# Sabarna07-tech/Multimodal-RAG-for-Image-Text-Search

Measured on AMD Instinct MI355X. Metric: CLIP img-embeds/sec/GPU; kNN queries/sec on 1M×512 at top-k=10, 1/2/4/8 GPUs, higher is better.
Workload: dtype fp16 MFMA scan + f64 exact rescore; 1 GPU; BASELINE config 3 (N=1) / config 4 (N>1): brute-force cosine top-10, 1M x 512 rows per GPU, 1000-query batch; rows_per_gpu=1048576, total_rows=1048576, dim=512, top_k=10, parallelism=row-sharded x1, uncertified_queries_last_step=0, searches_in_flight=2

## Files before the change

multimodal-rag-for-image-text-search_amd/csrc/knn.hip:

```cpp
#include <algorithm>
#include <cstdlib>
#include <mutex>
#include <shared_mutex>
#include <type_traits>
#include <utility>
#include <vector>

#include "common.h"
#include "knn_generic.h"

#define AS1 __attribute__((address_space(1)))
#define AS3 __attribute__((address_space(3)))

namespace {

constexpr int TILE_ROWS = 64;
constexpr int SCAN_WAVES = 8;
constexpr int SCAN_THREADS = SCAN_WAVES * 64;
constexpr int QPW = 32;
constexpr int QPG = SCAN_WAVES * QPW;
constexpr int MAX_MERGE_ENTRIES = 4096;
constexpr int MAX_K = 256;
constexpr int MERGE_THREADS = 256;
#ifndef MRAG_SAMPLE_STRIDE
#define MRAG_SAMPLE_STRIDE 16
#endif
constexpr int SAMPLE_STRIDE = MRAG_SAMPLE_STRIDE;

constexpr double EPS_F16 = 1.05e-3;

struct ScanParams {
  const _Float16* x16;
  const int32_t* labels;
  const _Float16* q16;
  int ntiles, qgroups, splits, Qp, label_filter;
  float* part_s;
  int32_t* part_i;
  const int32_t* fail_list;
  const int32_t* fail_cnt;
  const float* thresh;
  int32_t* cand_cnt;
  int32_t* cand;
  int ccap;
  uint32_t* theta;
  int sample_tiles, sample_stride;
  int k;
  float* part_tau;
};

template <int KL>
__device__ __forceinline__ void list_insert(float (&ls)[KL], int (&li)[KL], float s, int r) {
  float cs = s;
  int cr = r;
#pragma unroll
  for (int j = 0; j < KL; ++j) {
    const bool sw = cs > ls[j];
    const float ts = ls[j];
    const int tr = li[j];
    ls[j] = sw ? cs : ts;
    li[j] = sw ? cr : tr;
    cs = sw ? ts : cs;
    cr = sw ? tr : cr;
  }
}

template <int KL>
__device__ __forceinline__ void list_insert_par(float (&ls)[KL], int (&li)[KL], float s, int r) {
  bool c[KL];
#pragma unroll
  for (int j = 0; j < KL; ++j) c[j] = s > ls[j];
  float ns[KL];
  int ni[KL];
  ns[0] = c[0] ? s : ls[0];
  ni[0] = c[0] ? r : li[0];
#pragma unroll
  for (int j = 1; j < KL; ++j) {
    ns[j] = c[j] ? (c[j - 1] ? ls[j - 1] : s) : ls[j];
    ni[j] = c[j] ? (c[j - 1] ? li[j - 1] : r) : li[j];
  }
#pragma unroll
  for (int j = 0; j < KL; ++j) {
    ls[j] = ns[j];
    li[j] = ni[j];
  }
}

__device__ __forceinline__ void glds_x4(const void* gsrc, uint32_t lds_addr) {
  unsigned keep;
  asm volatile(
      "s_mov_b32 %0, m0\n\ts_mov_b32 m0, %2\n\ts_nop 0\n\tglobal_load_lds_dwordx4 %1, off\n\ts_mov_b32 m0, %0"
      : "=&s"(keep)
      : "v"(gsrc), "s"(lds_addr)
      : "memory");
}
__device__ __forceinline__ void glds_x4_saddr(uint32_t voff, const void* sbase, uint32_t lds_addr) {
  unsigned keep;
  asm volatile(
      "s_mov_b32 %0, m0\n\ts_mov_b32 m0, %3\n\ts_nop 0\n\tglobal_load_lds_dwordx4 %1, %2\n\ts_mov_b32 m0, %0"
      : "=&s"(keep)
      : "v"(voff), "s"(sbase), "s"(lds_addr)
// ... 281 lines not shown
    } else {
      qg = b % p.qgroups;
      split = b / p.qgroups;
    }
  }
  const int slot0 = qg * QPG3 + w * QPW3 + c16;

  half8 qf[KSTEPS][QB];
#pragma unroll
  for (int kk = 0; kk < KSTEPS; ++kk)
#pragma unroll
    for (int qb = 0; qb < QB; ++qb)
      qf[kk][qb] = *(const half8*)(p.q16 + (size_t)(slot0 + 16 * qb) * DP + kk * 32 + g4 * 8);
#pragma unroll
  for (int kk = 0; kk < KSTEPS; ++kk)
#pragma unroll
    for (int qb = 0; qb < QB; ++qb) asm volatile("" ::"a"(qf[kk][qb]));

  float ls[QB][KL3];
  int li[QB][KL3];
  float theta_f[QB], published[QB];
  float thr[QB];
  uint32_t theta_next[QB];
#pragma unroll
  for (int qb = 0; qb < QB; ++qb) {
#pragma unroll
    for (int j = 0; j < KL3; ++j) {
      ls[qb][j] = -INFINITY;
      li[qb][j] = -1;
    }
    theta_f[qb] = -INFINITY;
    thr[qb] = -INFINITY;
    published[qb] = -INFINITY;
    theta_next[qb] = 0u;
  }
  uint32_t* const theta_q = p.theta + slot0;
  const bool may_publish = p.k <= KL3;
  const int lab_lo = p.label_filter == MRAG_LABEL_ANY ? 0 : p.label_filter;
  const uint32_t lab_span = p.label_filter == MRAG_LABEL_ANY ? 0x7fffffffu : 0u;

  const int offA0_init = c16 * ROW_BYTES + 16 * (g4 ^ c16);

  f32x4 acc[2][4][QB];
#pragma unroll
  for (int i = 0; i < 4; ++i)
#pragma unroll
    for (int j = 0; j < QB; ++j) {
      acc[1][i][j] = f32x4{-INFINITY, -INFINITY, -INFINITY, -INFINITY};
      acc[0][i][j] = f32x4{};
    }

  int my_tiles = (split < p.ntiles) ? (p.ntiles - 1 - split) / p.splits + 1 : 0;
  int tstep = p.splits;
  if constexpr (MODE == 1) {
    my_tiles = min(my_tiles, p.sample_tiles);
    tstep = p.splits * p.sample_stride;
  }
  float smax[QB];
#pragma unroll
  for (int qb = 0; qb < QB; ++qb) smax[qb] = -INFINITY;

  auto stage_piece = [&](int buf, int tile, int i, int lane_t) {
    const char* gt = (const char*)p.x16 + (size_t)tile * TILE_BYTES;
    const unsigned piece = w * GLDS_PER_WAVE + i;
    const unsigned P = piece * 64 + (unsigned)lane_t;
    const unsigned row = P / CPR;
    const unsigned pos = P - row * CPR;
    const unsigned c = pos ^ (row & 15);
    glds_x4(gt + row * ROW_BYTES + c * 16, lds_base + buf * TILE_BYTES + piece * 1024);
  };
  auto stage_labels = [&](int buf, int tile) {
    if (w == 0) glds_x1(p.labels + (size_t)tile * TILE_ROWS + lane, lds_base + LBL_OFF + buf * TILE_ROWS * 4);
  };

  int prow = 0;
#ifdef MRAG_K7_STAMPS
  unsigned long long st_sum[7] = {0, 0, 0, 0, 0, 0, 0}, st_mid = 0;
#endif
  auto epi_group = [&](auto g_c, auto y_c) {
    constexpr int G = decltype(g_c)::value;
    constexpr int Y = decltype(y_c)::value;
    constexpr int qb = G >> 2, rb = G & 3;
    f32x4& av = acc[Y][rb][qb];
    float gm;
    asm("v_max3_f32 %0, %1, %2, %3\n\tv_max_f32 %0, %0, %4"
        : "=&v"(gm)
        : "v"(av[0]), "v"(av[1]), "v"(av[2]), "v"(av[3]));
    if constexpr (MODE == 1) {
      float sm = smax[qb];
      asm volatile("v_max_f32 %0, %0, %1" : "+v"(sm) : "v"(gm));
      smax[qb] = sm;
    } else {
      if (__builtin_expect(__any(gm > thr[qb]), 0)) {
#ifdef MRAG_K7_STAMPS
        const unsigned long long fire_t0 = __builtin_amdgcn_s_memtime();
#endif
#pragma unroll
        for (int r = 0; r < 4; ++r) {
          const float sv = av[r];
          if (sv > fmaxf(ls[qb][KL3 - 1], theta_f[qb]))
            list_insert_par<KL3>(ls[qb], li[qb], sv, prow + 16 * rb + r);
        }
        if (may_publish && li[qb][KL3 - 1] >= 0 && ls[qb][KL3 - 1] > published[qb]) {
          published[qb] = ls[qb][KL3 - 1];
          __hip_atomic_fetch_max(theta_q + 16 * qb, mrag_f2ord(published[qb]), __ATOMIC_RELAXED,
                                 __HIP_MEMORY_SCOPE_AGENT);
        }
        thr[qb] = fmaxf(ls[qb][KL3 - 1], theta_f[qb]);
#ifdef MRAG_K7_STAMPS
        st_sum[5] += 1;
        st_sum[6] += __builtin_amdgcn_s_memtime() - fire_t0;
#endif
      }
    }
  };

  constexpr int NA = QB == 4 ? 5 : 4;
  half8 a[NA];
  const int offA0 = offA0_init;
  auto read_a = [&](const char* tb, int kk, int rb) {
    a[(4 * kk + rb) % NA] =
        *(const half8*)(tb + ((offA0 ^ ((kk & 3) << 6)) + (kk >> 2) * 256 + rb * 16 * ROW_BYTES));
  };

  uint32_t m0_keep = 0;
#ifdef MRAG_K7_STAMPS
  unsigned long long st_end[3] = {0, 0, 0};
#endif
  auto end_of_tile = [&](bool wait_part) {
    if (!wait_part) {
#ifdef MRAG_K7_STAMPS
      st_end[0] = __builtin_amdgcn_s_memtime();
#endif
      if constexpr (CPR == 64 && QB == 4) asm volatile("s_mov_b32 m0, %0" ::"s"(m0_keep));
    }
    if (wait_part) {
      asm volatile("s_waitcnt vmcnt(0)" ::: "memory");
      if constexpr (MODE == 0) {
        if (may_publish) {
#pragma unroll
          for (int qb = 0; qb < QB; ++qb) {
            if (theta_next[qb] != 0) theta_f[qb] = fmaxf(theta_f[qb], mrag_ord2f(theta_next[qb]));
            thr[qb] = fmaxf(ls[qb][KL3 - 1], theta_f[qb]);
            asm volatile("" : "+v"(theta_f[qb]), "+v"(thr[qb]));
          }
        }
      }
#ifdef MRAG_K7_STAMPS
      st_end[1] = __builtin_amdgcn_s_memtime();
#endif
      __syncthreads();
#ifdef MRAG_K7_STAMPS
      st_end[2] = __builtin_amdgcn_s_memtime();
#endif
    }
  };

  auto tile_body = [&](auto x_c, int it) {
    constexpr int X = decltype(x_c)::value;
    constexpr int Y = 1 - X;
    K7_STAMP(st0);
    const int tile = split + it * tstep;
    const bool has_next = it + 1 < my_tiles;
    const int ntile = has_next ? tile + tstep : tile;
    const char* gw = (const char*)p.x16 + (size_t)ntile * TILE_BYTES + (size_t)w * GLDS_PER_WAVE * ROW_BYTES;
    uint32_t ldsw = lds_base + Y * TILE_BYTES + w * GLDS_PER_WAVE * 1024;
    asm volatile("" : "+s"(gw), "+s"(ldsw));
    if constexpr (MODE == 0) {
      if (may_publish) {
#pragma unroll
        for (int qb = 0; qb < QB; ++qb)
          theta_next[qb] = __hip_atomic_load(theta_q + 16 * qb, __ATOMIC_RELAXED, __HIP_MEMORY_SCOPE_AGENT);
      }
    }
    const char* tb = smem + X * TILE_BYTES;
    int lane_t = lane;
    uint32_t lane16 = lane * 16;
    asm volatile("" : "+v"(lane_t), "+v"(lane16));
    uint32_t voff = 0;
    if constexpr (CPR == 64 && QB == 4) asm volatile("s_mov_b32 %0, m0" : "=s"(m0_keep));
#pragma unroll
    for (int n = 0; n < NA; ++n) read_a(tb, n >> 2, n & 3);
    stage_labels(Y, ntile);
    constexpr int KLAB = KSTEPS / 2 - 1;
    int lab_v = 0;
    uint64_t tile_mask = ~0ull;
    if constexpr (QB == 1) {
#pragma unroll
      for (int i = 0; i < GLDS_PER_WAVE; ++i) stage_piece(Y, ntile, i, lane_t);
      static_for<KSTEPS>([&](auto kk_c) {
        constexpr int kk = decltype(kk_c)::value;
        static_for<4>([&](auto rb_c) {
          constexpr int rb = decltype(rb_c)::value;
          if constexpr (kk == 0)
            mfma16_ab0(acc[X][rb][0], a[(4 * kk + rb) % NA], qf[kk][0]);
          else
            mfma16_ab(acc[X][rb][0], a[(4 * kk + rb) % NA], qf[kk][0]);
          if constexpr (kk + 1 < KSTEPS) read_a(tb, kk + 1, rb);
          if constexpr (kk == 0) epi_group(std::integral_constant<int, rb>{}, std::integral_constant<int, Y>{});
          __builtin_amdgcn_sched_barrier(0);
        });
      });
    } else static_for<KSTEPS>([&](auto kk_c) {
      constexpr int kk = decltype(kk_c)::value;
      constexpr int g0 = (kk * NGROUPS + KSTEPS - 1) / KSTEPS;
      constexpr int g1 = ((kk + 1) * NGROUPS + KSTEPS - 1) / KSTEPS;
      static_for<16>([&](auto j_c) {
        constexpr int j = decltype(j_c)::value;
        constexpr int rb = j >> 2, qb = j & 3;
        constexpr int n = 4 * kk + rb;
        if constexpr (kk == 0)
          mfma16_ab0(acc[X][rb][qb], a[n % NA], qf[kk][qb]);
        else
          mfma16_ab(acc[X][rb][qb], a[n % NA], qf[kk][qb]);
        if constexpr ((j & 3) == 3) {
          if constexpr (n + NA < 4 * KSTEPS) read_a(tb, (n + NA) >> 2, (n + NA) & 3);
        } else if constexpr ((j & 3) == 1) {
          constexpr int pc = FRONT * kk + (j >> 2);
          if constexpr (CPR == 64 && (j >> 2) < FRONT && pc < GLDS_PER_WAVE) {
            voff = (lane16 ^ (uint32_t)(pc << 4)) + (uint32_t)(pc * 1024);
            asm volatile("s_mov_b32 m0, %1" : "+v"(voff) : "s"(ldsw + pc * 1024));
          }
          static_assert(KLAB * FRONT >= GLDS_PER_WAVE, "label slots must follow the DMA k-steps");
          if constexpr (kk == KLAB && j == 1) lab_v = ((const int*)(smem + LBL_OFF + X * TILE_ROWS * 4))[lane];
          if constexpr (kk == KLAB + 1 && j == 1) tile_mask = __ballot((uint32_t)(lab_v - lab_lo) <= lab_span);
        } else if constexpr ((j & 3) == 2) {
          constexpr int pc = FRONT * kk + (j >> 2);
          if constexpr ((j >> 2) < FRONT && pc < GLDS_PER_WAVE) {
            if constexpr (CPR == 64)
              asm volatile("global_load_lds_dwordx4 %0, %1" ::"v"(voff), "s"(gw) : "memory");
            else
              stage_piece(Y, ntile, pc, lane_t);
          }
        } else if constexpr ((j & 3) == 0) {
          if constexpr (g0 + (j >> 2) < g1)
            epi_group(std::integral_constant<int, g0 + (j >> 2)>{}, std::integral_constant<int, Y>{});
        }
#ifdef MRAG_K7_STAMPS
        if constexpr (kk == (GLDS_PER_WAVE + FRONT - 1) / FRONT - 1 && j == 15) st_mid = __builtin_amdgcn_s_memtime();
#endif
        __builtin_amdgcn_sched_barrier(0);
      });
    });
    end_of_tile(false);
    if constexpr (QB == 1) {
      lab_v = ((const int*)(smem + LBL_OFF + X * TILE_ROWS * 4))[lane];
      tile_mask = __ballot((uint32_t)(lab_v - lab_lo) <= lab_span);
    }
    if (tile_mask != ~0ull) {
      mfma16_guard(acc[X]);
      const uint64_t lm = tile_mask >> (4 * g4);
#pragma unroll
      for (int rb = 0; rb < 4; ++rb)
#pragma unroll
        for (int r = 0; r < 4; ++r) {
          const bool ok = (lm >> (16 * rb + r)) & 1ull;
#pragma unroll
          for (int qb = 0; qb < QB; ++qb) acc[X][rb][qb][r] = ok ? acc[X][rb][qb][r] : -INFINITY;
        }
    }
    prow = tile * TILE_ROWS + 4 * g4;
    end_of_tile(true);
#ifdef MRAG_K7_STAMPS
    if constexpr (QB == 4) {
      st_sum[0] += st_mid - st0;
      st_sum[1] += st_end[0] - st_mid;
    } else {
      st_sum[1] += st_end[0] - st0;
    }
    st_sum[2] += st_end[1] - st_end[0];
    st_sum[3] += st_end[2] - st_end[1];
    st_sum[4] += 1;
#endif
  };

  if constexpr (MODE == 0) {
    if (!may_publish) {
#pragma unroll
      for (int qb = 0; qb < QB; ++qb) {
        const uint32_t t0 = __hip_atomic_load(theta_q + 16 * qb, __ATOMIC_RELAXED, __HIP_MEMORY_SCOPE_AGENT);
        if (t0 != 0) theta_f[qb] = mrag_ord2f(t0);
        thr[qb] = theta_f[qb];
      }
    }
  }
  if (my_tiles > 0) {
#pragma unroll
    for (int i = 0; i < GLDS_PER_WAVE; ++i) stage_piece(0, split, i, lane);
    stage_labels(0, split);
    asm volatile("s_waitcnt vmcnt(0)" ::: "memory");
    __syncthreads();
    for (int it = 0; it < my_tiles; it += 2) {
      tile_body(std::integral_constant<int, 0>{}, it);
      if (it + 1 < my_tiles) tile_body(std::integral_constant<int, 1>{}, it + 1);
    }
    if (my_tiles & 1) {
      static_for<NGROUPS>([&](auto g_c) { epi_group(g_c, std::integral_constant<int, 0>{}); });
    } else {
      static_for<NGROUPS>([&](auto g_c) { epi_group(g_c, std::integral_constant<int, 1>{}); });
    }
  }
#ifdef MRAG_K7_STAMPS
  if constexpr (MODE == 0) {
    const int wid = blockIdx.x * SCAN2_WAVES + w;
    if (lane == 0 && wid < K7_MAXWAVES)
      for (int i = 0; i < 7; ++i) g_k7_stamps[(size_t)wid * K7_NSTAMP + i] = st_sum[i];
  }
#endif

  if constexpr (MODE == 1) {
#pragma unroll
    for (int qb = 0; qb < QB; ++qb) {
      p.part_s[((size_t)split * p.Qp + slot0 + 16 * qb) * 4 + g4] = smax[qb];
    }
    return;
  }
#pragma unroll
  for (int qb = 0; qb < QB; ++qb) {
    float fs[8];
    int fi[8];
#pragma unroll
    for (int j = 0; j < 8; ++j) {
      fs[j] = j < KL3 ? ls[qb][j] : -INFINITY;
      fi[j] = j < KL3 ? li[qb][j] : -1;
    }
    float tau = li[qb][KL3 - 1] >= 0 ? ls[qb][KL3 - 1] : -INFINITY;
#pragma unroll
    for (int o = 16; o < 64; o += 16) {
#pragma unroll
      for (int j = 0; j < KL3; ++j) {
        const float ps = __shfl_xor(ls[qb][j], o);
        const int pi = __shfl_xor(li[qb][j], o);
        if (pi >= 0 && ps > fs[7]) list_insert<8>(fs, fi, ps, pi);
      }
      const int plast = __shfl_xor(li[qb][KL3 - 1], o);
      const float pl = __shfl_xor(ls[qb][KL3 - 1], o);
      if (plast >= 0) tau = fmaxf(tau, pl);
    }
    if (g4 == 0) {
      const int slot = slot0 + 16 * qb;
      float* os = p.part_s + ((size_t)split * p.Qp + slot) * 8;
      int32_t* oi = p.part_i + ((size_t)split * p.Qp + slot) * 8;
#pragma unroll
      for (int j = 0; j < 8; ++j) {
        os[j] = fs[j];
        oi[j] = fi[j];
      }
      if (fi[7] >= 0) tau = fmaxf(tau, fs[7]);
      p.part_tau[(size_t)split * p.Qp + slot] = tau;
    }
  }
}

constexpr float THETA_SEED_MARGIN = (float)(2.5 * EPS_F16);
__global__ __launch_bounds__(64) void theta_init_kernel(const float* __restrict__ smax, int nvals, int Qp, int k,
                                                        uint32_t* __restrict__ theta) {
  constexpr int PER_LANE = 16;
  const int q = blockIdx.x, lane = threadIdx.x;
  float v[PER_LANE];
  const int splits = nvals / 4;
#pragma unroll
  for (int t = 0; t < 4; ++t) {
    const int sp = lane + 64 * t;
    const f32x4 x = sp < splits ? *(const f32x4*)(smax + ((size_t)sp * Qp + q) * 4)
                                : f32x4{-INFINITY, -INFINITY, -INFINITY, -INFINITY};
#pragma unroll
    for (int u = 0; u < 4; ++u) v[4 * t + u] = x[u];
  }
  float kth = -INFINITY;
  for (int r = 0; r < k; ++r) {
    float best = -INFINITY;
    int bt = 0;
#pragma unroll
    for (int t = 0; t < PER_LANE; ++t)
      if (v[t] > best) {
        best = v[t];
        bt = t;
      }
    float wbest = best;
#pragma unroll
    for (int off = 32; off > 0; off >>= 1) wbest = fmaxf(wbest, __shfl_xor(wbest, off));
    if (wbest == -INFINITY) {
      kth = -INFINITY;
      break;
    }
    const uint64_t holders = __ballot(best == wbest);
    if (lane == (int)__builtin_ctzll(holders)) {
#pragma unroll
      for (int t = 0; t < PER_LANE; ++t)
        if (t == bt) v[t] = -INFINITY;
    }
    kth = wbest;
  }
  if (lane == 0) theta[q] = (kth == -INFINITY) ? 0u : mrag_f2ord(kth - THETA_SEED_MARGIN);
}

using mrag_knn::exact_cosine16;

struct MergeParams {
  const float* part_s;
  const int32_t* part_i;
  int splits, KL, Qp, nq, k, M, R, Mp;
  const float* q32;
  const double* qn;
  const float* x32;
  const double* xn;
  int D, DP;
  float* out_s;
  double* out_s64;
  int64_t* out_r;
  int64_t row_offset;
  float* thresh;
  int32_t* fail_list;
  int32_t* fail_cnt;
  int32_t* host_fail;
  const uint32_t* theta;
  const float* part_tau;
};

__device__ __forceinline__ float f32_round_down(double x) {
  float f = (float)x;
  if ((double)f > x) f = nextafterf(f, -INFINITY);
  return f;
}

template <int P>
__device__ __forceinline__ void wave_sort_keys(uint64_t (&k)[P], int lane) {
  constexpr int E = 64 * P;
#pragma unroll
  for (int size = 2; size <= E; size <<= 1) {
#pragma unroll
    for (int st = size >> 1; st > 0; st >>= 1) {
      if (st >= 64) {
        if constexpr (P == 2) {
          const uint64_t a = k[0], b = k[1];
          k[0] = a < b ? a : b;
          k[1] = a < b ? b : a;
        }
      } else {
#pragma unroll
        for (int pp = 0; pp < P; ++pp) {
          const int e = 64 * pp + lane;
          const bool asc = (e & size) == 0, lower = (lane & st) == 0;
          const uint64_t o = __shfl_xor((unsigned long long)k[pp], st);
          const uint64_t lo = k[pp] < o ? k[pp] : o, hi = k[pp] < o ? o : k[pp];
          k[pp] = (lower == asc) ? lo : hi;
        }
      }
    }
  }
}
template <int P>
__device__ __forceinline__ void wave_merge_lowest(uint64_t (&run)[P], const uint64_t (&b)[P], int lane) {
#pragma unroll
  for (int pp = 0; pp < P; ++pp) {
    const uint64_t rb = __shfl((unsigned long long)b[P - 1 - pp], 63 - lane);
    run[pp] = run[pp] < rb ? run[pp] : rb;
  }
#pragma unroll
  for (int st = 32 * P; st > 0; st >>= 1) {
    if (st >= 64) {
      if constexpr (P == 2) {
        const uint64_t a = run[0], c = run[1];
        run[0] = a < c ? a : c;
        run[1] = a < c ? c : a;
      }
    } else {
#pragma unroll
      for (int pp = 0; pp < P; ++pp) {
        const uint64_t o = __shfl_xor((unsigned long long)run[pp], st);
        const bool lower = (lane & st) == 0;
        run[pp] = lower ? (run[pp] < o ? run[pp] : o) : (run[pp] < o ? o : run[pp]);
      }
    }
  }
}

#ifdef MRAG_K7_STAMPS
constexpr int K8_NSTAMP = 8, K8_MAXBLK = 4096;
__device__ unsigned long long g_k8_stamps[K8_MAXBLK * K8_NSTAMP];
#define K8_STAMP(i) k8t[i] = __builtin_amdgcn_s_memtime()
#else
#define K8_STAMP(i)
#endif
template <int SEL>
__global__ __launch_bounds__(MERGE_THREADS) void knn_merge_kernel(MergeParams p) {
  extern __shared__ __attribute__((aligned(16))) char dsm[];
  uint64_t* keys = (uint64_t*)dsm;
  double* ex = (double*)(dsm + (size_t)p.R * 8);
  int32_t* er = (int32_t*)(dsm + (size_t)p.R * 8 + (size_t)p.Mp * 8);
  float* qs = (float*)(dsm + (size_t)p.R * 8 + (size_t)p.Mp * 12);
  float* red_f = (float*)(dsm + (size_t)p.R * 8 + (size_t)p.Mp * 12 + (size_t)p.DP * 4);
  int* red_i = (int*)(red_f + MERGE_THREADS / 64);

  const int q = blockIdx.x;
  const int tid = threadIdx.x, lane = tid & 63, wave = tid >> 6;
#ifdef MRAG_K7_STAMPS
  unsigned long long k8t[K8_NSTAMP] = {};
#endif
  K8_STAMP(0);

  float tau = -INFINITY;
  int valid = 0;
  const int ntot = p.splits * p.KL;
  struct Raw {
    int r;
    float s;
  };
  auto load_raw = [&](int e) -> Raw {
    const int ec = e < ntot ? e : 0;
    const int sp = ec / p.KL, j = ec - sp * p.KL;
    const size_t o = ((size_t)sp * p.Qp + q) * p.KL + j;
    return Raw{p.part_i[o], p.part_s[o]};
  };
  auto make_key = [&](int e, Raw v) -> uint64_t {
    if (e >= ntot || v.r < 0) return ~0ull;
    ++valid;
    if (e % p.KL == p.KL - 1) tau = fmaxf(tau, v.s);
    return ((uint64_t)(~mrag_f2ord(v.s)) << 32) | (uint32_t)v.r;
  };
  auto load_key = [&](int e) -> uint64_t { return make_key(e, load_raw(e)); };
  if (p.part_tau)
    for (int sp = tid; sp < p.splits; sp += MERGE_THREADS) tau = fmaxf(tau, p.part_tau[(size_t)sp * p.Qp + q]);
  for (int d = tid; d < p.DP; d += MERGE_THREADS) qs[d] = p.q32[(size_t)q * p.DP + d];
  if constexpr (SEL == 0) {
    for (int e = tid; e < p.R; e += MERGE_THREADS) keys[e] = load_key(e);
  } else {
    constexpr int E = 64 * SEL;
    uint64_t run[SEL];
#pragma unroll
    for (int pp = 0; pp < SEL; ++pp) run[pp] = ~0ull;
    constexpr int NW = MERGE_THREADS / 64;
    Raw nx[SEL];
#pragma unroll
    for (int pp = 0; pp < SEL; ++pp) nx[pp] = load_raw(wave * E + 64 * pp + lane);
    for (int c = wave; c * E < ntot; c += NW) {
      uint64_t ch[SEL];
#pragma unroll
      for (int pp = 0; pp < SEL; ++pp) {
        ch[pp] = make_key(c * E + 64 * pp + lane, nx[pp]);
        nx[pp] = load_raw((c + NW) * E + 64 * pp + lane);
      }
      wave_sort_keys<SEL>(ch, lane);
      wave_merge_lowest<SEL>(run, ch, lane);
    }
#pragma unroll
    for (int pp = 0; pp < SEL; ++pp) keys[wave * E + 64 * pp + lane] = run[pp];
  }
  K8_STAMP(1);
#pragma unroll
  for (int off = 32; off > 0; off >>= 1) {
    tau = fmaxf(tau, __shfl_xor(tau, off));
    valid += __shfl_xor(valid, off);
  }
  if (lane == 0) {
    red_f[wave] = tau;
    red_i[wave] = valid;
  }
  __syncthreads();
  tau = red_f[0];
  valid = red_i[0];
  for (int i = 1; i < MERGE_THREADS / 64; ++i) {
    tau = fmaxf(tau, red_f[i]);
    valid += red_i[i];
  }

  if constexpr (SEL == 0) {
    for (int size = 2; size <= p.R; size <<= 1) {
      for (int stride = size >> 1; stride > 0; stride >>= 1) {
        __syncthreads();
        for (int i = tid; i < (p.R >> 1); i += MERGE_THREADS) {
// ... 371 lines not shown
  size_t bytes = 0;
};

int ensure(DevBuf& b, size_t bytes) {
  if (b.bytes >= bytes && b.p) return MRAG_OK;
  if (b.p) {
    MRAG_HIP(hipFree(b.p));
    b.p = nullptr;
    b.bytes = 0;
  }
  const size_t want = std::max<size_t>(bytes, 256);
  MRAG_HIP(hipMalloc(&b.p, want));
  b.bytes = want;
  return MRAG_OK;
}

void release(DevBuf& b) {
  if (b.p) (void)hipFree(b.p);
  b.p = nullptr;
  b.bytes = 0;
}

typedef void (*scan_fn)(ScanParams);

template <int DP>
scan_fn pick_scan(int KL, bool collect) {
  if (collect) return knn_scan_kernel<DP, 8, true>;
  if constexpr (DP >= 512) {
    return knn_scan_kernel<DP, 8, false>;
  } else if constexpr (DP >= 256) {
    return KL <= 8 ? knn_scan_kernel<DP, 8, false> : knn_scan_kernel<DP, 16, false>;
  } else {
    return KL <= 8 ? knn_scan_kernel<DP, 8, false>
                   : (KL <= 16 ? knn_scan_kernel<DP, 16, false> : knn_scan_kernel<DP, 32, false>);
  }
}

int kl_for(int k, int DP) {
  if (k <= 8 || DP >= 512) return 8;
  if (k <= 16 || DP >= 256) return 16;
  return 32;
}

template <int MODE, int QB>
scan_fn get_scan3m(int DP) {
  switch (DP) {
    case 128: return knn_scan3_kernel<128, MODE, QB>;
    case 256: return knn_scan3_kernel<256, MODE, QB>;
    case 384: return knn_scan3_kernel<384, MODE, QB>;
    case 512: return knn_scan3_kernel<512, MODE, QB>;
    default: return nullptr;
  }
}
scan_fn get_scan3(int DP, bool sample, int qb) {
  if (qb == 1) return sample ? nullptr : get_scan3m<0, 1>(DP);
  return sample ? get_scan3m<1, 4>(DP) : get_scan3m<0, 4>(DP);
}

int scan3_qb(int64_t nq) { return nq <= 64 ? 1 : 4; }

int sample_stride_for(int k) { return k > 16 ? 4 : SAMPLE_STRIDE; }

scan_fn get_scan(int DP, int KL, bool collect) {
  switch (DP) {
    case 128: return pick_scan<128>(KL, collect);
    case 256: return pick_scan<256>(KL, collect);
    case 384: return pick_scan<384>(KL, collect);
    case 512: return pick_scan<512>(KL, collect);
    default: return nullptr;
  }
}

int64_t next_pow2(int64_t x) {
  int64_t p = 1;
  while (p < x) p <<= 1;
  return p;
}

}

struct SearchCtx {
  DevBuf qin, q32, qn, q16, part_s, part_i, thresh, fail_list, counters, cand_cnt, cand, scratch;
  DevBuf out_s, out_s64, out_r, theta, part_tau;
  int32_t* host_counters = nullptr;
  int32_t* host_fail = nullptr;
  hipEvent_t done = nullptr;
  hipEvent_t null_ev = nullptr;
  hipEvent_t ev0 = nullptr, ev1 = nullptr;
  mrag_knn::Workspace gws[8];
};

struct mrag_knn_index {
  std::mutex mu;
  std::shared_mutex rw;
  int device = 0;
  int D = 0, DP = 0;
  int64_t n = 0, cap = 0;
  DevBuf x16, x32, xn, labels;
  hipStream_t stream = nullptr;
  DevBuf stage_rows, stage_labels, rowlist;
  std::mutex pool_mu;
  std::vector<SearchCtx*> ctx_all, ctx_free;
  int64_t last_uncertified = 0, last_retries = 0;
  SearchCtx* last_ctx = nullptr;
  int32_t last_info[8] = {0, 0, 0, 0, 0, 0, 0, 0};
  bool profile = false;
  double scan_ms = 0.0;
  int64_t scan_launches = 0;
};

namespace {

int wait_stream(SearchCtx* c, hipStream_t s) {
  MRAG_HIP(hipEventRecord(c->done, s));
  hipError_t e;
  while ((e = hipEventQuery(c->done)) == hipErrorNotReady) {
  }
  if (e != hipSuccess) return mrag::fail(MRAG_ERR_HIP, "search: %s", hipGetErrorString(e));
  return MRAG_OK;
}

void ctx_free_all(SearchCtx* c) {
  for (DevBuf* b : {&c->qin, &c->q32, &c->qn, &c->q16, &c->part_s, &c->part_i, &c->thresh, &c->fail_list,
                    &c->counters, &c->cand_cnt, &c->cand, &c->scratch, &c->out_s, &c->out_s64, &c->out_r,
                    &c->theta, &c->part_tau})
    release(*b);
  mrag_knn::release(c->gws);
  if (c->host_counters) (void)hipHostFree(c->host_counters);
  if (c->host_fail) (void)hipHostFree(c->host_fail);
  if (c->done) (void)hipEventDestroy(c->done);
  if (c->null_ev) (void)hipEventDestroy(c->null_ev);
  if (c->ev0) (void)hipEventDestroy(c->ev0);
  if (c->ev1) (void)hipEventDestroy(c->ev1);
  delete c;
}

int ctx_get(mrag_knn_index* ix, SearchCtx** out) {
  {
    std::lock_guard<std::mutex> lk(ix->pool_mu);
    if (!ix->ctx_free.empty()) {
      *out = ix->ctx_free.back();
      ix->ctx_free.pop_back();
      return MRAG_OK;
    }
  }
  auto* c = new SearchCtx();
  hipError_t e = hipHostMalloc((void**)&c->host_counters, 16, hipHostMallocDefault);
  if (e == hipSuccess) e = hipHostMalloc((void**)&c->host_fail, 16, hipHostMallocCoherent);
  if (e == hipSuccess) e = hipEventCreateWithFlags(&c->done, hipEventDisableTiming);
  if (e == hipSuccess) e = hipEventCreateWithFlags(&c->null_ev, hipEventDisableTiming);
  if (e == hipSuccess) e = hipEventCreate(&c->ev0);
  if (e == hipSuccess) e = hipEventCreate(&c->ev1);
  if (e != hipSuccess) {
    ctx_free_all(c);
    return mrag::fail(MRAG_ERR_HIP, "search context: %s", hipGetErrorString(e));
  }
  std::lock_guard<std::mutex> lk(ix->pool_mu);
  ix->ctx_all.push_back(c);
  *out = c;
  return MRAG_OK;
}

struct CtxLease {
  mrag_knn_index* ix;
  SearchCtx* c;
  ~CtxLease() {
    std::lock_guard<std::mutex> lk(ix->pool_mu);
    ix->ctx_free.push_back(c);
  }
};

int grow(mrag_knn_index* ix, int64_t need) {
  if (need <= ix->cap) return MRAG_OK;
  int64_t ncap = std::max<int64_t>({(int64_t)TILE_ROWS, ix->cap * 2, need});
  ncap = (ncap + 767) / 768 * 768;
  DevBuf nx16, nx32, nxn, nlab;
  if (int rc = ensure(nx16, (size_t)ncap * ix->DP * 2)) return rc;
  if (int rc = ensure(nx32, (size_t)ncap * ix->DP * 4)) return rc;
// ... 218 lines not shown

  auto generic_args = [&]() {
    mrag_knn::GenericSearch ga{};
    ga.x16 = (const _Float16*)ix->x16.p;
    ga.x32 = (const float*)ix->x32.p;
    ga.xn = (const double*)ix->xn.p;
    ga.labels = (const int32_t*)ix->labels.p;
    ga.n = ix->n;
    ga.D = D;
    ga.DP = DP;
    ga.q16 = (const _Float16*)c->q16.p;
    ga.q32 = (const float*)c->q32.p;
    ga.qn = (const double*)c->qn.p;
    ga.nq = (int)nq;
    ga.k = k;
    ga.label_filter = label_filter;
    ga.row_offset = row_offset;
    ga.out_s = os;
    ga.out_s64 = os64;
    ga.out_r = orr;
    return ga;
  };

  if (ix->n == 0) {
    hipLaunchKernelGGL(fill_empty_kernel, dim3((unsigned)((nout + 255) / 256)), dim3(256), 0, s, os, os64,
                       orr, nout);
    MRAG_CHECK_LAUNCH();
  } else if (DP > 512 || k > MAX_K) {
    const float* qsrc = queries;
    if (host) {
      if (int rc = ensure(c->qin, (size_t)nq * D * 4)) return rc;
      MRAG_HIP(hipMemcpyAsync(c->qin.p, queries, (size_t)nq * D * 4, hipMemcpyHostToDevice, s));
      qsrc = (const float*)c->qin.p;
    }
    if (int rc = ensure(c->q32, (size_t)nq * DP * 4)) return rc;
    if (int rc = ensure(c->qn, (size_t)nq * 8)) return rc;
    if (int rc = ensure(c->q16, (size_t)nq * DP * 2)) return rc;
    if (int rc = launch_prep(qsrc, nq, D, DP, nq, (float*)c->q32.p, (double*)c->qn.p, (_Float16*)c->q16.p, s))
      return rc;
    if (int rc = mrag_knn::search_generic(generic_args(), c->gws, s, nullptr)) return rc;
  } else {
    const bool use_v3 = k <= 64;
    const int qb = use_v3 ? scan3_qb(nq) : 4;
    const int qpg = use_v3 ? 64 * qb : QPG;
    const int64_t qpad = use_v3 ? qpg : QPW;
    const int64_t Qp = (nq + qpad - 1) / qpad * qpad;
    const int qgroups = (int)((Qp + qpg - 1) / qpg);
    const int ntiles = (int)((ix->n + TILE_ROWS - 1) / TILE_ROWS);
    const int KL = use_v3 ? 8 : kl_for(k, DP);
    int S = std::max(1, 256 / qgroups);
    S = std::min(S, ntiles);
    S = std::min(S, MAX_MERGE_ENTRIES / KL);
    if (S >= 8) S &= ~7;
    const int M = std::min<int>(k + 32, S * KL);
    const int R = (int)next_pow2((int64_t)S * KL);
    const int Mp = (int)next_pow2(std::max(M, 2));
    info[0] = S;
    info[1] = (int32_t)Qp;
    info[7] = KL;

    const float* qsrc = queries;
    if (host) {
      if (int rc = ensure(c->qin, (size_t)nq * D * 4)) return rc;
      MRAG_HIP(hipMemcpyAsync(c->qin.p, queries, (size_t)nq * D * 4, hipMemcpyHostToDevice, s));
      qsrc = (const float*)c->qin.p;
    }
    if (int rc = ensure(c->q32, (size_t)Qp * DP * 4)) return rc;
    if (int rc = ensure(c->qn, (size_t)Qp * 8)) return rc;
    if (int rc = ensure(c->q16, (size_t)Qp * DP * 2)) return rc;
    if (int rc = ensure(c->part_s, (size_t)S * Qp * KL * 4)) return rc;
    if (int rc = ensure(c->part_i, (size_t)S * Qp * KL * 4)) return rc;
    if (int rc = ensure(c->thresh, (size_t)Qp * 4)) return rc;
    if (int rc = ensure(c->fail_list, (size_t)Qp * 4)) return rc;
    if (int rc = ensure(c->counters, 16)) return rc;
    if (int rc = ensure(c->cand_cnt, (size_t)Qp * 4)) return rc;
    if (int rc = ensure(c->theta, (size_t)Qp * 4)) return rc;
    if (use_v3)
      if (int rc = ensure(c->part_tau, (size_t)S * Qp * 4)) return rc;

    if (int rc = launch_prep(qsrc, nq, D, DP, Qp, (float*)c->q32.p, (double*)c->qn.p, (_Float16*)c->q16.p, s,
                             PrepClear{(int32_t*)c->counters.p, (int32_t*)c->cand_cnt.p, (uint32_t*)c->theta.p}))
      return rc;

    ScanParams sp{};
    sp.theta = (uint32_t*)c->theta.p;

    sp.x16 = (const _Float16*)ix->x16.p;
    sp.labels = (const int32_t*)ix->labels.p;
    sp.q16 = (const _Float16*)c->q16.p;
    sp.ntiles = ntiles;
    sp.qgroups = qgroups;
    sp.splits = S;
    sp.Qp = (int)Qp;
    sp.label_filter = label_filter;
    sp.part_s = (float*)c->part_s.p;
    sp.part_i = (int32_t*)c->part_i.p;
    sp.fail_list = (const int32_t*)c->fail_list.p;
    sp.fail_cnt = (const int32_t*)c->counters.p;
    sp.thresh = (const float*)c->thresh.p;
    sp.cand_cnt = (int32_t*)c->cand_cnt.p;
    sp.k = k;
    sp.part_tau = use_v3 ? (float*)c->part_tau.p : nullptr;

    const scan_fn scan = use_v3 ? get_scan3(DP, false, qb) : get_scan(DP, KL, false);
    const scan_fn collect = get_scan(DP, 8, true);
    if (!scan || !collect) return mrag::fail(MRAG_ERR_UNSUPPORTED, "no scan kernel for DP=%d", DP);
    const dim3 sgrid((unsigned)(qgroups * S));
    const int min_tiles = ntiles / S;
    const int stride = sample_stride_for(k);
    if (use_v3 && qb == 4 && min_tiles >= 4 * stride) {
      sp.sample_stride = stride;
      sp.sample_tiles = min_tiles / stride;
      hipLaunchKernelGGL(get_scan3(DP, true, qb), sgrid, dim3(SCAN2_THREADS), 0, s, sp);
      MRAG_CHECK_LAUNCH();
      hipLaunchKernelGGL(theta_init_kernel, dim3((unsigned)nq), dim3(64), 0, s, (const float*)sp.part_s, 4 * S,
                         (int)Qp, k, sp.theta);
      MRAG_CHECK_LAUNCH();
    }
    if (profile) MRAG_HIP(hipEventRecord(c->ev0, s));
    hipLaunchKernelGGL(scan, sgrid, dim3(use_v3 ? SCAN2_THREADS : SCAN_THREADS), 0, s, sp);
    MRAG_CHECK_LAUNCH();
    if (profile) MRAG_HIP(hipEventRecord(c->ev1, s));

    MergeParams mp{};
    mp.part_s = sp.part_s;
    mp.part_i = sp.part_i;
    mp.splits = S;
    mp.KL = KL;
    mp.Qp = (int)Qp;
    mp.nq = (int)nq;
    mp.k = k;
    mp.M = M;
    mp.R = R;
    mp.Mp = Mp;
    mp.q32 = (const float*)c->q32.p;
    mp.qn = (const double*)c->qn.p;
    mp.x32 = (const float*)ix->x32.p;
    mp.xn = (const double*)ix->xn.p;
    mp.D = D;
    mp.DP = DP;
    mp.out_s = os;
    mp.out_s64 = os64;
    mp.out_r = orr;
    mp.row_offset = row_offset;
    mp.thresh = (float*)c->thresh.p;
    mp.fail_list = (int32_t*)c->fail_list.p;
    mp.fail_cnt = (int32_t*)c->counters.p;
    mp.theta = (const uint32_t*)c->theta.p;
    mp.part_tau = sp.part_tau;
    mp.host_fail = c->host_fail;
    __atomic_store_n(c->host_fail, 0, __ATOMIC_RELAXED);
    const int sel = M + 1 <= 64 ? 1 : (M + 1 <= 128 ? 2 : 0);
    mp.R = sel ? std::max(R, 4 * 64 * sel) : R;
    const size_t msh = (size_t)mp.R * 8 + (size_t)Mp * 12 + (size_t)DP * 4 + 64;
    auto merge = sel == 1 ? knn_merge_kernel<1> : sel == 2 ? knn_merge_kernel<2> : knn_merge_kernel<0>;
    hipLaunchKernelGGL(merge, dim3((unsigned)nq), dim3(MERGE_THREADS), msh, s, mp);
    MRAG_CHECK_LAUNCH();

    if (int rc = wait_stream(c, s)) return rc;
    if (__atomic_load_n(c->host_fail, __ATOMIC_ACQUIRE)) {
      MRAG_HIP(hipMemcpyAsync(c->host_counters, c->counters.p, 8, hipMemcpyDeviceToHost, s));
      if (int rc = wait_stream(c, s)) return rc;
    } else {
      c->host_counters[0] = 0;
    }
    if (profile) {
      float ms = 0.f;
      MRAG_HIP(hipEventElapsedTime(&ms, c->ev0, c->ev1));
      std::lock_guard<std::mutex> lk(ix->pool_mu);
      ix->scan_ms += ms;
      ix->scan_launches++;
    }
    uncertified = c->host_counters[0];
    if (uncertified > 0) {
      const int ccap = (int)std::max<int64_t>(256, std::min<int64_t>(4096, ((int64_t)64 << 20) / Qp));
      if (int rc = ensure(c->cand, (size_t)Qp * ccap * 4)) return rc;
      if (int rc = ensure(c->scratch, (size_t)Qp * ccap * 8)) return rc;
      sp.cand = (int32_t*)c->cand.p;
      sp.ccap = ccap;
      const int cgroups = (int)((uncertified + QPG - 1) / QPG);
// ... 92 lines not shown
```

Baseline: 1.095 million queries/s (1000-query batches, each query scanned against a 1M x 512 shard per GPU, top-10; aggregate over GPUs).

## Resolve sampled tiles exactly in a pre-pass and skip them in the main scan

Adds a counting sample mode in which the sample scan covers every stride-th tile and records, per query group, the top three packed score/id maxima. A new resolve kernel uses these to derive theta, recomputes dot products for the qualifying row groups of the sampled tiles, and writes extra partial lists for the merge. The main scan then skips the already-sampled tiles through a magic-number division in the tile index. This removes the duplicate scanning of sampled tiles and seeds a tighter threshold, at the cost of an extra kernel, more merge entries, and more complex tile indexing and tau handling.

```diff
diff --git a/multimodal-rag-for-image-text-search_amd/csrc/knn.hip b/multimodal-rag-for-image-text-search_amd/csrc/knn.hip
--- a/multimodal-rag-for-image-text-search_amd/csrc/knn.hip
+++ b/multimodal-rag-for-image-text-search_amd/csrc/knn.hip
@@ -46,6 +46,9 @@
   int sample_tiles, sample_stride;
   int k;
   float* part_tau;
+  uint32_t* rec;
+  uint32_t rec_keep;
+  uint32_t skip_magic;
 };
 
 template <int KL>
@@ -433,13 +436,29 @@
 
   int my_tiles = (split < p.ntiles) ? (p.ntiles - 1 - split) / p.splits + 1 : 0;
   int tstep = p.splits;
+  uint32_t skip_magic = 0u;
+  int skip_off = 0;
   if constexpr (MODE == 1) {
     my_tiles = min(my_tiles, p.sample_tiles);
     tstep = p.splits * p.sample_stride;
-  }
+  } else if constexpr (MODE == 2) {
+    my_tiles = (my_tiles + p.sample_stride - 1) / p.sample_stride;
+    tstep = p.splits * p.sample_stride;
+  } else if constexpr (QB == 4) {
+    if (p.skip_magic != 0u) {
+      my_tiles -= (my_tiles + p.sample_stride - 1) / p.sample_stride;
+      skip_magic = p.skip_magic;
+      skip_off = 1;
+    }
+  }
+  auto tile_of = [&](int it) { return split + (it + (int)__umulhi((uint32_t)it, skip_magic) + skip_off) * tstep; };
   float smax[QB];
 #pragma unroll
   for (int qb = 0; qb < QB; ++qb) smax[qb] = -INFINITY;
+  uint32_t rm1[QB], rm2[QB], rm3[QB];
+#pragma unroll
+  for (int qb = 0; qb < QB; ++qb) rm1[qb] = rm2[qb] = rm3[qb] = 0u;
+  int pid = 0;
 
   auto stage_piece = [&](int buf, int tile, int i, int lane_t) {
     const char* gt = (const char*)p.x16 + (size_t)tile * TILE_BYTES;
@@ -463,6 +482,16 @@
     constexpr int Y = decltype(y_c)::value;
     constexpr int qb = G >> 2, rb = G & 3;
     f32x4& av = acc[Y][rb][qb];
+    if constexpr (MODE == 2) {
+      const int gmi = max(max(max(__float_as_int(av[0]), __float_as_int(av[1])), __float_as_int(av[2])),
+                          max(__float_as_int(av[3]), 0));
+      const uint32_t v = ((uint32_t)gmi & p.rec_keep) | (uint32_t)(pid + rb);
+      const uint32_t m1 = rm1[qb], m2 = rm2[qb];
+      rm3[qb] = max(rm3[qb], min(v, m2));
+      asm("v_med3_u32 %0, %1, %2, %3" : "=v"(rm2[qb]) : "v"(v), "v"(m1), "v"(m2));
+      rm1[qb] = max(m1, v);
+      return;
+    }
     float gm;
     asm("v_max3_f32 %0, %1, %2, %3\n\tv_max_f32 %0, %0, %4"
         : "=&v"(gm)
@@ -541,9 +570,9 @@
     constexpr int X = decltype(x_c)::value;
     constexpr int Y = 1 - X;
     K7_STAMP(st0);
-    const int tile = split + it * tstep;
+    const int tile = tile_of(it);
     const bool has_next = it + 1 < my_tiles;
-    const int ntile = has_next ? tile + tstep : tile;
+    const int ntile = has_next ? tile_of(it + 1) : tile;
     const char* gw = (const char*)p.x16 + (size_t)ntile * TILE_BYTES + (size_t)w * GLDS_PER_WAVE * ROW_BYTES;
     uint32_t ldsw = lds_base + Y * TILE_BYTES + w * GLDS_PER_WAVE * 1024;
     asm volatile("" : "+s"(gw), "+s"(ldsw));
@@ -641,6 +670,7 @@
         }
     }
     prow = tile * TILE_ROWS + 4 * g4;
+    if constexpr (MODE == 2) pid = 4 * it;
     end_of_tile(true);
 #ifdef MRAG_K7_STAMPS
     if constexpr (QB == 4) {
@@ -667,8 +697,8 @@
   }
   if (my_tiles > 0) {
 #pragma unroll
-    for (int i = 0; i < GLDS_PER_WAVE; ++i) stage_piece(0, split, i, lane);
-    stage_labels(0, split);
+    for (int i = 0; i < GLDS_PER_WAVE; ++i) stage_piece(0, tile_of(0), i, lane);
+    stage_labels(0, tile_of(0));
     asm volatile("s_waitcnt vmcnt(0)" ::: "memory");
     __syncthreads();
     for (int it = 0; it < my_tiles; it += 2) {
@@ -693,6 +723,15 @@
 #pragma unroll
     for (int qb = 0; qb < QB; ++qb) {
       p.part_s[((size_t)split * p.Qp + slot0 + 16 * qb) * 4 + g4] = smax[qb];
+    }
+    return;
+  }
+  if constexpr (MODE == 2) {
+#pragma unroll
+    for (int qb = 0; qb < QB; ++qb) {
+      using u32x4 = uint32_t __attribute__((ext_vector_type(4)));
+      *(u32x4*)(p.rec + (((size_t)split * p.Qp + slot0 + 16 * qb) * 4 + g4) * 4) =
+          u32x4{rm1[qb], rm2[qb], rm3[qb], 0u};
     }
     return;
   }
@@ -776,12 +815,144 @@
   if (lane == 0) theta[q] = (kth == -INFINITY) ? 0u : mrag_f2ord(kth - THETA_SEED_MARGIN);
 }
 
+struct ResolveParams {
+  const uint32_t* rec;
+  uint32_t idmask;
+  int splits, Qp, k, DP, tile_step, label_filter;
+  const _Float16* x16;
+  const _Float16* q16;
+  const int32_t* labels;
+  uint32_t* theta;
+  float* part_s;
+  int32_t* part_i;
+  float* part_tau;
+};
+constexpr int XLISTS = 4, XCAP = XLISTS * 8;
+constexpr int REC_ID_BITS_MAX = 10;
+
+__global__ __launch_bounds__(64) void sample_resolve_kernel(ResolveParams p) {
+  using u32x4 = uint32_t __attribute__((ext_vector_type(4)));
+  constexpr int PER_LANE = 32;
+  __shared__ uint32_t qrec[64 * PER_LANE];
+  __shared__ float xs[XCAP + 16];
+  __shared__ int xr[XCAP + 16];
+  const int q = blockIdx.x, lane = threadIdx.x;
+  const uint64_t lt = (1ull << lane) - 1;
+  uint32_t u[PER_LANE], m3 = 0u;
+#pragma unroll
+  for (int t = 0; t < 4; ++t) {
+    const int sp = lane + 64 * t;
+#pragma unroll
+    for (int g = 0; g < 4; ++g) {
+      const u32x4 r = sp < p.splits ? *(const u32x4*)(p.rec + (((size_t)sp * p.Qp + q) * 4 + g) * 4)
+                                    : u32x4{0u, 0u, 0u, 0u};
+      u[8 * t + 2 * g] = r[0];
+      u[8 * t + 2 * g + 1] = r[1];
+      m3 = max(m3, r[2]);
+    }
+  }
+#pragma unroll
+  for (int off = 32; off > 0; off >>= 1) m3 = max(m3, (uint32_t)__shfl_xor((int)m3, off));
+
+  uint32_t kth = 0u, prev = ~0u;
+  int above = 0;
+  for (int r = 0; r < p.k; ++r) {
+    uint32_t best = 0u;
+    int c = 0;
+#pragma unroll
+    for (int i = 0; i < PER_LANE; ++i) best = max(best, u[i] < prev ? u[i] : 0u);
+#pragma unroll
+    for (int off = 32; off > 0; off >>= 1) best = max(best, (uint32_t)__shfl_xor((int)best, off));
+    if (best <= p.idmask) break;
+#pragma unroll
+    for (int i = 0; i < PER_LANE; ++i) c += u[i] == best;
+#pragma unroll
+    for (int off = 32; off > 0; off >>= 1) c += __shfl_xor(c, off);
+    above += c;
+    if (above >= p.k) {
+      kth = best;
+      break;
+    }
+    prev = best;
+  }
+  float theta_f = -INFINITY;
+  if (kth != 0u) theta_f = __uint_as_float(kth & ~p.idmask) - THETA_SEED_MARGIN;
+  if (lane == 0) p.theta[q] = kth != 0u ? mrag_f2ord(theta_f) : 0u;
+
+  int nrec = 0;
+#pragma unroll
+  for (int i = 0; i < PER_LANE; ++i) {
+    const bool qf = u[i] > p.idmask && __uint_as_float(u[i] | p.idmask) > theta_f;
+    const uint64_t b = __ballot(qf);
+    if (qf)
+      qrec[nrec + __popcll(b & lt)] =
+          ((uint32_t)(lane + 64 * (i >> 3)) << 12) | ((uint32_t)((i >> 1) & 3) << 10) | (u[i] & p.idmask);
+    nrec += __popcll(b);
+  }
+  __syncthreads();
+
+  const int lab_lo = p.label_filter == MRAG_LABEL_ANY ? 0 : p.label_filter;
+  const uint32_t lab_span = p.label_filter == MRAG_LABEL_ANY ? 0x7fffffffu : 0u;
+  const int gsel = lane >> 4, rr = (lane >> 2) & 3, sub = lane & 3;
+  const half8* qrow = (const half8*)(p.q16 + (size_t)q * p.DP);
+  int cnt = 0;
+  float tau_drop = -INFINITY;
+  for (int base = 0; base < nrec; base += 4) {
+    const bool have = base + gsel < nrec;
+    const uint32_t pk = qrec[have ? base + gsel : base];
+    const int sp = (int)(pk >> 12), g = (int)(pk >> 10) & 3, id = (int)(pk & p.idmask);
+    const int64_t row = (int64_t)(sp + (id >> 2) * p.tile_step) * TILE_ROWS + 16 * (id & 3) + 4 * g + rr;
+    const half8* xrow = (const half8*)(p.x16 + row * p.DP);
+    float acc = 0.f;
+    for (int c = sub; c < p.DP / 8; c += 4) {
+      const half8 a = xrow[c], b = qrow[c];
+#pragma unroll
+      for (int e = 0; e < 8; ++e) acc += (float)a[e] * (float)b[e];
+    }
+    acc += __shfl_xor(acc, 1);
+    acc += __shfl_xor(acc, 2);
+    const int lab = p.labels[row];
+    const bool take = have && sub == 0 && (uint32_t)(lab - lab_lo) <= lab_span && acc > theta_f;
+    const uint64_t b = __ballot(take);
+    if (take) {
+      const int pos = cnt + __popcll(b & lt);
+      xs[pos] = acc;
+      xr[pos] = (int)row;
+    }
+    cnt += __popcll(b);
+    __syncthreads();
+    while (cnt > XCAP) {
+      const float v = lane < cnt ? xs[lane] : INFINITY;
+      float wmin = v;
+#pragma unroll
+      for (int off = 32; off > 0; off >>= 1) wmin = fminf(wmin, __shfl_xor(wmin, off));
+      const int holder = (int)__builtin_ctzll(__ballot(v == wmin));
+      tau_drop = fmaxf(tau_drop, wmin);
+      if (lane == 0) {
+        xs[holder] = xs[cnt - 1];
+        xr[holder] = xr[cnt - 1];
+      }
+      --cnt;
+      __syncthreads();
+    }
+  }
+  if (lane < XCAP) {
+    const size_t o = ((size_t)(p.splits + lane / 8) * p.Qp + q) * 8 + (lane & 7);
+    p.part_s[o] = lane < cnt ? xs[lane] : -INFINITY;
+    p.part_i[o] = lane < cnt ? xr[lane] : -1;
+  }
+  if (lane < XLISTS)
+    p.part_tau[(size_t)(p.splits + lane) * p.Qp + q] =
+        lane == 0 ? fmaxf(__uint_as_float(m3 | p.idmask), tau_drop) : -INFINITY;
+}
+
 using mrag_knn::exact_cosine16;
 
 struct MergeParams {
   const float* part_s;
   const int32_t* part_i;
   int splits, KL, Qp, nq, k, M, R, Mp;
+  int scan_splits;
   const float* q32;
   const double* qn;
   const float* x32;
@@ -883,7 +1054,7 @@
 
   float tau = -INFINITY;
   int valid = 0;
-  const int ntot = p.splits * p.KL;
+  const int ntot = p.splits * p.KL, nscan = p.scan_splits * p.KL;
   struct Raw {
     int r;
     float s;
@@ -897,7 +1068,7 @@
   auto make_key = [&](int e, Raw v) -> uint64_t {
     if (e >= ntot || v.r < 0) return ~0ull;
     ++valid;
-    if (e % p.KL == p.KL - 1) tau = fmaxf(tau, v.s);
+    if (e % p.KL == p.KL - 1 && e < nscan) tau = fmaxf(tau, v.s);
     return ((uint64_t)(~mrag_f2ord(v.s)) << 32) | (uint32_t)v.r;
   };
   auto load_key = [&](int e) -> uint64_t { return make_key(e, load_raw(e)); };
@@ -1375,14 +1546,15 @@
     default: return nullptr;
   }
 }
-scan_fn get_scan3(int DP, bool sample, int qb) {
-  if (qb == 1) return sample ? nullptr : get_scan3m<0, 1>(DP);
-  return sample ? get_scan3m<1, 4>(DP) : get_scan3m<0, 4>(DP);
+scan_fn get_scan3(int DP, int mode, int qb) {
+  if (qb == 1) return mode ? nullptr : get_scan3m<0, 1>(DP);
+  return mode == 2 ? get_scan3m<2, 4>(DP) : mode == 1 ? get_scan3m<1, 4>(DP) : get_scan3m<0, 4>(DP);
 }
 
 int scan3_qb(int64_t nq) { return nq <= 64 ? 1 : 4; }
 
 int sample_stride_for(int k) { return k > 16 ? 4 : SAMPLE_STRIDE; }
+bool counting_sample_for(int k) { return k <= 16; }
 
 scan_fn get_scan(int DP, int KL, bool collect) {
   switch (DP) {
@@ -1404,7 +1576,7 @@
 
 struct SearchCtx {
   DevBuf qin, q32, qn, q16, part_s, part_i, thresh, fail_list, counters, cand_cnt, cand, scratch;
-  DevBuf out_s, out_s64, out_r, theta, part_tau;
+  DevBuf out_s, out_s64, out_r, theta, part_tau, rec;
   int32_t* host_counters = nullptr;
   int32_t* host_fail = nullptr;
   hipEvent_t done = nullptr;
@@ -1446,7 +1618,7 @@
 void ctx_free_all(SearchCtx* c) {
   for (DevBuf* b : {&c->qin, &c->q32, &c->qn, &c->q16, &c->part_s, &c->part_i, &c->thresh, &c->fail_list,
                     &c->counters, &c->cand_cnt, &c->cand, &c->scratch, &c->out_s, &c->out_s64, &c->out_r,
-                    &c->theta, &c->part_tau})
+                    &c->theta, &c->part_tau, &c->rec})
     release(*b);
   mrag_knn::release(c->gws);
   if (c->host_counters) (void)hipHostFree(c->host_counters);
@@ -1771,8 +1943,16 @@
     S = std::min(S, ntiles);
     S = std::min(S, MAX_MERGE_ENTRIES / KL);
     if (S >= 8) S &= ~7;
+    const int min_tiles = ntiles / S;
+    const int stride = sample_stride_for(k);
+    const bool sampled = use_v3 && qb == 4 && min_tiles >= 4 * stride;
+    const int max_sample_tiles = ((ntiles + S - 1) / S + stride - 1) / stride;
+    int idbits = 2;
+    while ((1 << idbits) < 4 * max_sample_tiles) ++idbits;
+    const bool counting = sampled && counting_sample_for(k) && idbits <= REC_ID_BITS_MAX;
+    const int SX = counting ? XLISTS : 0;
     const int M = std::min<int>(k + 32, S * KL);
-    const int R = (int)next_pow2((int64_t)S * KL);
+    const int R = (int)next_pow2((int64_t)(S + SX) * KL);
     const int Mp = (int)next_pow2(std::max(M, 2));
     info[0] = S;
     info[1] = (int32_t)Qp;
@@ -1787,15 +1967,17 @@
     if (int rc = ensure(c->q32, (size_t)Qp * DP * 4)) return rc;
     if (int rc = ensure(c->qn, (size_t)Qp * 8)) return rc;
     if (int rc = ensure(c->q16, (size_t)Qp * DP * 2)) return rc;
-    if (int rc = ensure(c->part_s, (size_t)S * Qp * KL * 4)) return rc;
-    if (int rc = ensure(c->part_i, (size_t)S * Qp * KL * 4)) return rc;
+    if (int rc = ensure(c->part_s, (size_t)(S + SX) * Qp * KL * 4)) return rc;
+    if (int rc = ensure(c->part_i, (size_t)(S + SX) * Qp * KL * 4)) return rc;
     if (int rc = ensure(c->thresh, (size_t)Qp * 4)) return rc;
     if (int rc = ensure(c->fail_list, (size_t)Qp * 4)) return rc;
     if (int rc = ensure(c->counters, 16)) return rc;
     if (int rc = ensure(c->cand_cnt, (size_t)Qp * 4)) return rc;
     if (int rc = ensure(c->theta, (size_t)Qp * 4)) return rc;
     if (use_v3)
-      if (int rc = ensure(c->part_tau, (size_t)S * Qp * 4)) return rc;
+      if (int rc = ensure(c->part_tau, (size_t)(S + SX) * Qp * 4)) return rc;
+    if (counting)
+      if (int rc = ensure(c->rec, (size_t)S * Qp * 16 * 4)) return rc;
 
     if (int rc = launch_prep(qsrc, nq, D, DP, Qp, (float*)c->q32.p, (double*)c->qn.p, (_Float16*)c->q16.p, s,
                              PrepClear{(int32_t*)c->counters.p, (int32_t*)c->cand_cnt.p, (uint32_t*)c->theta.p}))
@@ -1821,19 +2003,42 @@
     sp.k = k;
     sp.part_tau = use_v3 ? (float*)c->part_tau.p : nullptr;
 
-    const scan_fn scan = use_v3 ? get_scan3(DP, false, qb) : get_scan(DP, KL, false);
+    const scan_fn scan = use_v3 ? get_scan3(DP, 0, qb) : get_scan(DP, KL, false);
     const scan_fn collect = get_scan(DP, 8, true);
     if (!scan || !collect) return mrag::fail(MRAG_ERR_UNSUPPORTED, "no scan kernel for DP=%d", DP);
     const dim3 sgrid((unsigned)(qgroups * S));
-    const int min_tiles = ntiles / S;
-    const int stride = sample_stride_for(k);
-    if (use_v3 && qb == 4 && min_tiles >= 4 * stride) {
-      sp.sample_stride = stride;
+    sp.sample_stride = stride;
+    if (sampled) {
       sp.sample_tiles = min_tiles / stride;
-      hipLaunchKernelGGL(get_scan3(DP, true, qb), sgrid, dim3(SCAN2_THREADS), 0, s, sp);
+      if (counting) {
+        sp.rec = (uint32_t*)c->rec.p;
+        sp.rec_keep = ~((1u << idbits) - 1u);
+      }
+      hipLaunchKernelGGL(get_scan3(DP, counting ? 2 : 1, qb), sgrid, dim3(SCAN2_THREADS), 0, s, sp);
       MRAG_CHECK_LAUNCH();
-      hipLaunchKernelGGL(theta_init_kernel, dim3((unsigned)nq), dim3(64), 0, s, (const float*)sp.part_s, 4 * S,
-                         (int)Qp, k, sp.theta);
+      if (counting) {
+        ResolveParams rp{};
+        rp.rec = sp.rec;
+        rp.idmask = ~sp.rec_keep;
+        rp.splits = S;
+        rp.Qp = (int)Qp;
+        rp.k = k;
+        rp.DP = DP;
+        rp.tile_step = S * stride;
+        rp.label_filter = label_filter;
+        rp.x16 = sp.x16;
+        rp.q16 = sp.q16;
+        rp.labels = sp.labels;
+        rp.theta = sp.theta;
+        rp.part_s = sp.part_s;
+        rp.part_i = sp.part_i;
+        rp.part_tau = sp.part_tau;
+        hipLaunchKernelGGL(sample_resolve_kernel, dim3((unsigned)nq), dim3(64), 0, s, rp);
+        sp.skip_magic = (uint32_t)((1ull << 32) / (uint64_t)(stride - 1) + 1);
+      } else {
+        hipLaunchKernelGGL(theta_init_kernel, dim3((unsigned)nq), dim3(64), 0, s, (const float*)sp.part_s, 4 * S,
+                           (int)Qp, k, sp.theta);
+      }
       MRAG_CHECK_LAUNCH();
     }
     if (profile) MRAG_HIP(hipEventRecord(c->ev0, s));
@@ -1844,7 +2049,8 @@
     MergeParams mp{};
     mp.part_s = sp.part_s;
     mp.part_i = sp.part_i;
-    mp.splits = S;
+    mp.splits = S + SX;
+    mp.scan_splits = S;
     mp.KL = KL;
     mp.Qp = (int)Qp;
     mp.nq = (int)nq;
```

Result: faster. 1.129 million queries/s (1000-query batches, each query scanned against a 1M x 512 shard per GPU, top-10; aggregate over GPUs), median of 6 (+3.0%).
